# osmocom/osmo-trx

Hardware: AMD Instinct MI355X
Metric: Mbursts/s detect+demod (156.25 sym, 4 SPS) (higher is better)
Workload: dtype f32

## Files before the change

### osmo_trx_amd/csrc/trx_kernel_nb.hip

```cpp
#include "trx_k4_common.h"
#include "trx_nb_asm.inc"

#define NB_D_LEN    160
#define NB_CZ_LEN   (TRX_CZ_PAD + TRX_CORR_NARROW + TRX_CZ_PAD)
#define NB_SLICE    (K4_XS + NB_D_LEN + NB_CZ_LEN)
#define NB_COMP_ROWS (TRX_DELAY_FILTS + 1)
#define NB_TABLES_FLOATS (TRX_SINCV_LDS + 16 * WAVE + NB_COMP_ROWS * 36 + 16 + 8 * 8 + 5 * WAVE + 5 * WAVE + 2 * 8 * 16)
#define NB_TABLES_BYTES (NB_TABLES_FLOATS * 4)
#define NB_WPB 16
#define NB_POOL_RING 64
#define NB_POOL_UNSET (-1)
#define NB_POOL_END (-2)
#define NB_NO_BURST 0xffffffffu
#define NB_LDS_TAIL (16 + 4 * NB_POOL_RING)
#define NB_LDS_BYTES (NB_TABLES_BYTES + NB_WPB * NB_SLICE * 8 + NB_LDS_TAIL)
#define NB_MAX_TOA 32



typedef float v3f __attribute__((ext_vector_type(3)));
typedef int v4i __attribute__((ext_vector_type(4)));
typedef __attribute__((address_space(3))) v2f lds_v2f;

template <typename T>
// ... 160 lines not shown

	uint32_t pre_i[NLD];
	uint32_t pre_prm = 0u;
	auto prefetch = [&](unsigned bb) {
		pre_prm = reinterpret_cast<const uint32_t *>(params)[2 * (size_t)bb];
		const char *src = reinterpret_cast<const char *>(iq + (size_t)bb * 625);
		const uint32_t *const row = reinterpret_cast<const uint32_t *>(src + a_l4);
#pragma unroll
		for (int r = 0; r < NLD - 1; r++)
			pre_i[r] = __builtin_nontemporal_load(row + r * WAVE);
		pre_i[NLD - 1] = __builtin_nontemporal_load(reinterpret_cast<const uint32_t *>(src + a_l4c) + (NLD - 1) * WAVE);
	};
	const unsigned b_first = burst_of((unsigned)wave);
	if (b_first != NB_NO_BURST)
		prefetch(b_first);

	v3f o = { 0.0f, 0.0f, 0.0f };
	int recw = 0;
	int pend_m = 0;
	int pend_rm = 0;
	unsigned pend_b = 0;
	int left_any = 0;
	auto store_pending = [&]() {
		float *const so = soft + (size_t)pend_b * 148;
		int *const rp = reinterpret_cast<int *>(results + pend_b);
		const float oe = o.x;
		asm volatile("s_bfm_b64 exec, 48, 2\n\t"
			     "s_and_b32 exec_lo, exec_lo, %7\n\t"
			     "s_and_b32 exec_hi, exec_hi, %7\n\t"
			     "global_store_dwordx3 %0, %1, %2\n\t"
			     "s_mov_b32 exec_lo, 0\n\t"
			     "s_and_b32 exec_hi, %7, 0x92400000\n\t"
			     "global_store_dword %0, %3, %2\n\t"
			     "s_mov_b32 exec_lo, %8\n\t"
			     "s_mov_b32 exec_hi, 0\n\t"
			     "global_store_dword %4, %5, %6\n\t"
			     "s_mov_b64 exec, -1\n\t"
			     "s_nop 0"
			     :: "v"(a_st), "v"(o), "s"(so), "v"(oe), "v"(a_l4), "v"(recw), "s"(rp), "s"(pend_m), "s"(pend_rm)
			     : "memory", "scc");
	};
	int q_xr = 0, q_xi = 0, q_es = 0, q_toa = 0, q_s = 0, q_fl = 0, q_b = 0;
	int q_n = 0;
	auto flush_records = [&]() {
		const int lane = nb_lane_id();
		if (lane < q_n) {
			const float *const h = lhdr + 8 * (q_fl & 0xff);
			const float xr = __int_as_float(q_xr), xi = __int_as_float(q_xi);
			const float a0 = xr * h[2], a1 = xr * h[3], a2 = xi * h[3], a3 = xi * h[2];
			const float amp_re = a0 - a2, amp_im = a1 + a3;
			const float toa = (float)q_toa * 0.001953125f;
			const float energy = __int_as_float(q_es) * 0.0125f;
			const float rssi = rssi_db(full_scale, energy);
			const float p2 = xi * xi + xr * xr;
			const float C = p2 * h[7];
			const float S = __int_as_float(q_s);
			const float ci = 3.0103f * __log2f(C * __builtin_amdgcn_rcpf(S - C));
			const v4i r0 = { 1, __float_as_int(toa), __float_as_int(amp_re), __float_as_int(amp_im) };
			const v4i r1 = { __float_as_int(ci), __float_as_int(energy), __float_as_int(rssi), q_fl };
			asm volatile("global_store_dwordx4 %0, %1, off\n\t"
				     "global_store_dwordx4 %0, %2, off offset:16\n\t"
				     "s_nop 1"
				     :: "v"(results + (unsigned)q_b), "v"(r0), "v"(r1) : "memory");
		}
		asm volatile("");
		q_n = 0;
	};

	auto queue_record = [&](const int xr_bits, const int xi_bits, const int es_bits, const int toa, const int s_bits, const int fl, const unsigned bb) {
		asm("s_lshl_b64 exec, 1, %[n]\n\t"
		    "v_mov_b32_e32 %[qxr], %[xr]\n\t"
		    "v_mov_b32_e32 %[qxi], %[xi]\n\t"
		    "v_mov_b32_e32 %[qes], %[es]\n\t"
		    "v_mov_b32_e32 %[qtoa], %[toa]\n\t"
		    "v_mov_b32_e32 %[qs], %[ss]\n\t"
		    "v_mov_b32_e32 %[qfl], %[fl]\n\t"
		    "v_mov_b32_e32 %[qb], %[b]\n\t"
		    "s_mov_b64 exec, -1"
		    : [qxr] "+v"(q_xr), [qxi] "+v"(q_xi), [qes] "+v"(q_es), [qtoa] "+v"(q_toa), [qs] "+v"(q_s), [qfl] "+v"(q_fl),
		      [qb] "+v"(q_b)
		    : [n] "s"(uni(q_n)), [xr] "s"(xr_bits), [xi] "s"(xi_bits), [es] "s"(es_bits), [toa] "s"(toa),
		      [ss] "s"(s_bits), [fl] "s"(fl), [b] "s"((int)bb)
		    : "scc");
		q_n++;
	};

	auto demod_general = [&](const int nk, const c32 ampv, const int lane) -> bool {
		constexpr int L = 625, nwrite = 148;
		c32 *const dec = D;
		const trx_tables *tabc = reinterpret_cast<const trx_tables *>(e8_addr - offsetof(trx_tables, edge8));
		asm volatile("" : "+s"(tabc));
		const int w = nk >> 7, fr = nk & 127;
		const int fidx = (fr >= 2) ? (fr >> 1) : TRX_DELAY_FILTS;
		const float ian = __builtin_amdgcn_rcpf(norm2(ampv));
		const c32 scale = make_float2(ampv.x * ian, -ampv.y * ian);
		const int n_lo = w > 0 ? w : 0;
		const int n_hi = (L - 1 + w < 623) ? L - 1 + w : 623;
		const int i_full_lo = cdiv4(n_lo + 15), i_full_hi = fdiv4(n_hi);
		const int i0l = cdiv4(n_lo), i0h = i_full_hi + 1;
		const bool need_lo = (n_hi >= n_lo) && (i0l < i_full_lo) && (i0l < nwrite);
		const bool need_hi = (n_hi >= n_lo) && (i0h <= fdiv4(n_hi + 15)) && (i0h < nwrite);
		if (uni((need_lo && !(n_hi >= 4 * (i_full_lo - 1))) || (need_hi && !((w <= -2) && (n_lo <= 4 * i0h - 15)))))
			return false;
		const int lo_tab = uni(need_lo);
		float ct0 = 0.0f, ct1 = 0.0f, ct2 = 0.0f;
		const int le = lane >> 4, lt = lane & 15;
		const int li = i0l + le;
		const int lt0 = n_lo + 15 - 4 * li;
		const bool lact = lt0 >= 1;
		if (lo_tab) {
			const float *row = &tabc->edge_lo[fidx][(lact ? lt0 : 1) - 1][lt];
			ct0 = row[0];
			ct1 = row[16];
			ct2 = (lt < 4) ? row[32] : 0.0f;
		}
		const int hi_tab = uni(need_hi);
		float ch0 = 0.0f, ch1 = 0.0f, ch2 = 0.0f;
		const int hi_i = i0h + le;
		const int htm = n_hi + 15 - 4 * hi_i;
		const bool hact = htm >= 0;
		if (hi_tab) {
			const float *row = &tabc->edge_hi[fidx][hact ? htm : 0][lt];
			ch0 = row[0];
			ch1 = row[16];
			ch2 = (lt < 4) ? row[32] : 0.0f;
		}
		int tabv = lo_tab | (hi_tab << 1);
		asm volatile("" : "+v"(tabv));
		{
			const int c_full = -24 - w;
			const int i_min = cdiv4(-36 - c_full), i_max = fdiv4(L + 1 - c_full);
			int ic = 3 * lane;
			if (ic < i_min) ic = i_min;
			if (ic > i_max - 2) ic = i_max - 2;
			v2f acc[3];
			asm volatile(NB_ASM_FIRG
				     : [a0] "=&v"(acc[0]), [a1] "=&v"(acc[1]), [a2] "=&v"(acc[2])
				     : [nk] "s"(nk), [pb] "s"(lds_addr(P)), [cb] "s"(lds_addr(comp) + 4u * (K4_U0 + TRX_FUSED_SH)), [kic] "v"(8 * ic)
				     : NB_ASM_CLOBBERS);
			if (n_lo == 0 && lo_tab && i_full_hi >= nwrite - 1) {
				if (lane < 52) {
#pragma unroll
					for (int j = 0; j < 3; j++)
						dec[3 * lane + j] = cmul(make_float2(acc[j].x, acc[j].y), scale);
				}
			} else {
#pragma unroll
				for (int j = 0; j < 3; j++) {
					const int i = 3 * lane + j;
					const bool full = (i >= i_full_lo) && (i <= i_full_hi);
					const c32 d = full ? cmul(make_float2(acc[j].x, acc[j].y), scale) : make_float2(0.0f, 0.0f);
					if (i < 156)
						dec[i] = d;
				}
			}
		}
		const int tab2 = uni(tabv), lo_tab2 = tab2 & 1, hi_tab2 = tab2 & 2;
		if (lo_tab2) {
			const int s0 = 4 * li - 24 - w + lt;
			const c32 *pp = P + ((s0 & 3) * PH_A + PH_M0 + (s0 >> 2));
			const c32 x0 = lds_c32(pp), x1 = lds_c32(pp + 4), x2 = lds_c32(pp + 8);
			float ar = x0.x * ct0, ai = x0.y * ct0;
			ar = fmaf(x1.x, ct1, ar); ai = fmaf(x1.y, ct1, ai);
			ar = fmaf(x2.x, ct2, ar); ai = fmaf(x2.y, ct2, ai);
			const float sr = row_sum(ar), si = row_sum(ai);
			int lt0s = lt0;
			asm volatile("" : "+v"(lt0s));
// ... 105 lines not shown
				int clip;
				asm("s_cmp_lg_u64 %1, 0\n\ts_cselect_b32 %0, 1, 0" : "=s"(clip) : "s"(__ballot(amax > TRX_CLIP_THRESH)) : "scc");

				const int len = 16 + (int)max_toa;
				__builtin_assume(len >= 16 && len <= 16 + NB_MAX_TOA);
				float v;
				const int lag0 = (len <= NB_ASM_CORR_MAX_LEN) ? NB_ASM_CORR_LANE0 : 0;
				asm volatile(NB_ASM_DECCORR
					     : [nrm] "=&v"(v)
					     : [aw] "v"(a_w), [zero] "v"(0), [len] "s"(len), [tsc] "s"(tsc)
					     : NB_ASM_CLOBBERS);
				{
					DIAG_MARK(3);
					int m_bits, es_bits, bidx;
					int kr, ka, kb, kic, ktp;
					asm volatile(NB_ASM_AMAX("ds_read_b32 %[kr], %[l4] offset:%c[lc]", "ds_read_b32 %[ka], %[l4] offset:%c[lc]+256",
								 "ds_read_b32 %[kb], %[l4] offset:%c[lc]+512", "ds_read_b32 %[kic], %[l4] offset:%c[lc]+768",
								 "ds_read_b32 %[ktp], %[l4] offset:%c[lc]+1024", "s_nop 0", "s_nop 0", "s_nop 0")
						     "s_sub_u32 %[bidx], %[bidx], %[lag0]\n\t"
						     "s_waitcnt lgkmcnt(0)"
						     : [m] "=&s"(m_bits), [es] "=&s"(es_bits), [bidx] "=&s"(bidx), [kr] "=&v"(kr), [ka] "=&v"(ka), [kb] "=&v"(kb),
						       [kic] "=&v"(kic), [ktp] "=&v"(ktp)
						     : [nrm] "v"(v), [ep] "v"(epart), [l4] "v"(a_l4), [lag0] "s"(lag0),
						       [lc] "n"((TRX_SINCV_LDS + 16 * WAVE + NB_COMP_ROWS * 36 + 16 + 64 + 5 * WAVE) * 4)
						     : NB_ASM_CLOBBERS);
					DIAG_MARK(4);
					int st, e512;
					float km;
					asm volatile(NB_ASM_DETA
						     : [st] "=&" NB_ASM_ST(st), [e] "=&s"(e512), [km] "=&v"(km)
						     : [bidx] "s"(bidx), [len] "s"(len), [czb] "s"(lds_addr(cz)), [kr] "v"(kr), [ka] "v"(ka), [l16] "v"(a_l16),
						       [gkv] "v"(gkv), [c0] "v"(gc0)
						     : NB_ASM_CLOBBERS_ST);
					DIAG_MARK(5);
					int toa512 = 0, xr_bits = 0, xi_bits = 0;
					if (__builtin_expect(st == 1, 1)) {
						asm volatile(NB_ASM_DETB
							     : [st] "=&" NB_ASM_ST(st), [toa] "=&s"(toa512), [xr] "=&s"(xr_bits), [xi] "=&s"(xi_bits)
							     : [e] "s"(e512), [kb] "v"(kb), [czb] "s"(lds_addr(cz)), [km] "v"(km)
							     : NB_ASM_CLOBBERS_ST);
						DIAG_MARK(6);
					}
					if (__builtin_expect(st != 1, 0)) {
						int stc = st;
						asm volatile("" : "+s"(stc));
						if (stc == 3) {
							const int lane = nb_lane_id();
							if (lane == 0)
								atomicAdd(&g_trx_fast_stats[0], 1ull);
							PeakConst pkc;
							pkc.flA = pkcl[0 * WAVE + lane]; pkc.loA = pkcl[1 * WAVE + lane]; pkc.hiA = pkcl[2 * WAVE + lane];
							pkc.offB = pkcl[3 * WAVE + lane]; pkc.ratio_off = pkcl[4 * WAVE + lane];
							c32 xcorr;
							peak_detect_spec(cz, bidx, sincv, pkc, lane, &toa512, &xcorr, wa4);
							toa512 = uni(toa512);
							xr_bits = uni(__float_as_int(xcorr.x));
							xi_bits = uni(__float_as_int(xcorr.y));
							st = 1;
						} else if (stc == 2) {
							if (nb_lane_id() == 0) atomicAdd(&g_trx_fast_stats[2], 1ull);
							mark_left(b);
							keep = 0;
						} else {
							const float energy = __int_as_float(es_bits) * 0.0125f;
							const float rssi = rssi_db(full_scale, energy);
							const uint32_t flags = ((uint32_t)clip << 8) | (1u << 16);
							int word = clip ? -TRXHIP_SIGERR_CLIP : 0;
							word = put_lane<1>(word, 0.0f);
							word = put_lane<2>(word, 0.0f);
							word = put_lane<3>(word, 0.0f);
							word = put_lane<4>(word, 0.0f);
							word = put_lane<5>(word, energy);
							word = put_lane<6>(word, rssi);
							word = write_lane<7>(word, (int)flags);
							recw = word;
							o = (v3f){ 0.0f, 0.0f, 0.0f };
							pend_rm = 0xff;
						}
					}
					if (__builtin_expect(st == 1, 1)) {
						int ok, s_bits;
						float d0, d1, d2;
						const int t5 = (t5pk << (28 - 4 * tsc)) >> 28;
						asm volatile("s_setprio 0");
						asm volatile(NB_ASM_TAIL
							     : [ok] "=&s"(ok), [ssum] "=&s"(s_bits), [d0] "=&v"(d0), [d1] "=&v"(d1), [d2] "=&v"(d2)
							     : [toa] "s"(toa512), [xr] "s"(xr_bits), [xi] "s"(xi_bits), [t5] "s"(t5), [hdrb] "s"(lds_addr(lhdr) + 32u * (unsigned)tsc),
							       [e8lo] "s"((unsigned)e8_addr), [e8hi] "s"((unsigned)(e8_addr >> 32)), [l16] "v"(a_l16),
							       [aw] "v"(a_w), [pb] "s"(lds_addr(P)), [cb] "s"(lds_addr(comp) + 4u * (K4_U0 + TRX_FUSED_SH)), [db] "s"(lds_addr(D)),
							       [kic] "v"(kic), [ktp] "v"(ktp)
							     : NB_ASM_CLOBBERS);
						DIAG_MARK(10);
						asm volatile("s_setprio 2");
						o.x = __builtin_amdgcn_fmed3f(fmaf(0.5f, d0, 0.5f), 0.0f, 1.0f);
						o.y = __builtin_amdgcn_fmed3f(fmaf(0.5f, d1, 0.5f), 0.0f, 1.0f);
						o.z = __builtin_amdgcn_fmed3f(fmaf(0.5f, d2, 0.5f), 0.0f, 1.0f);
						queue_record(xr_bits, xi_bits, es_bits, toa512 - t5 - 10 * 512, s_bits,
							     (int)((uint32_t)tsc | ((uint32_t)clip << 8) | (37u << 24)), b);
						if (__builtin_expect(!ok, 0)) {
							const int lane = nb_lane_id();
							if (lane == 0) atomicAdd(&g_trx_fast_stats[3], 1ull);
							const float *const h = lhdr + 8 * tsc;
							const float xr = __int_as_float(xr_bits), xi = __int_as_float(xi_bits);
							const float a0 = xr * h[2], a1 = xr * h[3], a2 = xi * h[3], a3 = xi * h[2];
							const c32 ampv = make_float2(unif(a0 - a2), unif(a1 + a3));
							if (!demod_general(t5 + 10 * 512 - toa512, ampv, lane)) {
								q_n--;
								mark_left(b);
								keep = 0;
							}
						}
					}
				}
			}
		}
		pend_b = b;
		pend_m = keep;
		if (__builtin_expect(q_n == WAVE, 0))
			flush_records();
		DIAG_MARK(11);
	}
	asm volatile(NB_ASM_COLD ::: NB_ASM_CLOBBERS);
	store_pending();
	flush_records();
	DIAG_FLUSH();
	if (pooled) {
		__syncthreads();
		int tid0;
		asm volatile("v_mbcnt_lo_u32_b32 %0, -1, 0\n\tv_mbcnt_hi_u32_b32 %0, -1, %0" : "=v"(tid0));
		if (tid0 == 0 && atomicAdd(wg_next + 1, 1) == 0) {
			const unsigned d = __hip_atomic_fetch_add(pool_ctr + 1, 1u, __ATOMIC_ACQ_REL, __HIP_MEMORY_SCOPE_AGENT);
			if (d == gridDim.x - 1u) {
				__hip_atomic_store(pool_ctr, 0u, __ATOMIC_RELAXED, __HIP_MEMORY_SCOPE_AGENT);
				__hip_atomic_store(pool_ctr + 1, 0u, __ATOMIC_RELEASE, __HIP_MEMORY_SCOPE_AGENT);
			}
		}
	}
}
```

### osmo_trx_amd/csrc/trx_nb_asm.inc

```
#define NB_ASM_GDEC_OFF 29968
#define NB_ASM_LSEQ_OFF 32848
#define NB_ASM_DEC_MAX_NACT 60
#define NB_ASM_CORR_LANE0 19
#define NB_ASM_CORR_MAX_LEN 45
#define NB_ASM_AW_PD 512
#define NB_ASM_AW_D 5760
#define NB_ASM_AW_CZ 7136
#define NB_ASM_ST "{s98}"
#define NB_ASM_CLOBBERS "v64", "v65", "v66", "v67", "v68", "v69", "v70", "v71", "v72", "v73", "v74", "v75", "v76", "v77", "v78", "v79", "v80", "v81", "v82", "v83", "v84", "v85", "v86", "v87", "v88", "v89", "v90", "v91", "v92", "v93", "v94", "v95", "v96", "v97", "v98", "v99", "v100", "v101", "v102", "v103", "v104", "v105", "v106", "v107", "v108", "v109", "v110", "v111", "v112", "v113", "v114", "v115", "v116", "v117", "v118", "v119", "v120", "v121", "v122", "v123", "v124", "v125", "v126", "v127", "s87", "s88", "s89", "s90", "s91", "s92", "s93", "s94", "s95", "s96", "s97", "s98", "s99", "vcc", "scc", "memory"
#define NB_ASM_CLOBBERS_ST "v64", "v65", "v66", "v67", "v68", "v69", "v70", "v71", "v72", "v73", "v74", "v75", "v76", "v77", "v78", "v79", "v80", "v81", "v82", "v83", "v84", "v85", "v86", "v87", "v88", "v89", "v90", "v91", "v92", "v93", "v94", "v95", "v96", "v97", "v98", "v99", "v100", "v101", "v102", "v103", "v104", "v105", "v106", "v107", "v108", "v109", "v110", "v111", "v112", "v113", "v114", "v115", "v116", "v117", "v118", "v119", "v120", "v121", "v122", "v123", "v124", "v125", "v126", "v127", "s87", "s88", "s89", "s90", "s91", "s92", "s93", "s94", "s95", "s96", "s97", "s99", "vcc", "scc", "memory"
#define NB_ASM_DECCORR \
	"s_add_u32 s92, %[len], 15\n\t" \
	"s_cmp_gt_u32 %[len], 45\n\t" \
	"s_cbranch_scc1 .Lnbc_dc_wide\n\t" \
	"s_sub_u32 s88, 60, s92\n\t" \
	"s_lshr_b64 exec, -1, s88\n\t" \
	"ds_read_b128 v[120:123], %[zero] offset:29968\n\t" \
	"ds_read_b128 v[124:127], %[zero] offset:29984\n\t" \
	"ds_read_b64 v[98:99], %[aw] offset:1952\n\t" \
	"ds_read_b64 v[100:101], %[aw] offset:3392\n\t" \
	"ds_read_b64 v[102:103], %[aw] offset:4832\n\t" \
	"ds_read_b64 v[96:97], %[aw] offset:512\n\t" \
	"s_waitcnt lgkmcnt(3)\n\t" \
	"v_pk_mul_f32 v[64:65], v[98:99], v[120:121] op_sel:[0,0] op_sel_hi:[1,0]\n\t" \
// ... 1320 lines not shown
	"v_pk_fma_f32 v[64:65], v[84:85], v[98:99], v[64:65] op_sel:[0,0,0] op_sel_hi:[1,0,1]\n\t" \
	"v_pk_fma_f32 v[66:67], v[86:87], v[98:99], v[66:67] op_sel:[0,1,0] op_sel_hi:[1,1,1]\n\t" \
	"ds_read_b64 v[108:109], v69 offset:80\n\t" \
	"ds_read_b32 v122, v72 offset:4096\n\t" \
	"ds_read_b64 v[110:111], v69 offset:88\n\t" \
	"ds_read_b32 v123, v72 offset:6144\n\t" \
	"s_waitcnt lgkmcnt(12)\n\t" \
	"v_pk_fma_f32 v[64:65], v[88:89], v[100:101], v[64:65] op_sel:[0,0,0] op_sel_hi:[1,0,1]\n\t" \
	"v_pk_fma_f32 v[66:67], v[90:91], v[100:101], v[66:67] op_sel:[0,1,0] op_sel_hi:[1,1,1]\n\t" \
	"ds_read_b64 v[112:113], v69 offset:96\n\t" \
	"ds_read_b32 v124, v72 offset:8192\n\t" \
	"ds_read_b64 v[114:115], v69 offset:104\n\t" \
	"ds_read_b32 v125, v72 offset:10240\n\t" \
	"s_waitcnt lgkmcnt(12)\n\t" \
	"v_pk_fma_f32 v[64:65], v[92:93], v[102:103], v[64:65] op_sel:[0,0,0] op_sel_hi:[1,0,1]\n\t" \
	"v_pk_fma_f32 v[66:67], v[94:95], v[102:103], v[66:67] op_sel:[0,1,0] op_sel_hi:[1,1,1]\n\t" \
	"ds_read_b64 v[116:117], v69 offset:112\n\t" \
	"ds_read_b32 v126, v72 offset:12288\n\t" \
	"ds_read_b64 v[118:119], v69 offset:120\n\t" \
	"ds_read_b32 v127, v72 offset:14336\n\t" \
	"s_waitcnt lgkmcnt(12)\n\t" \
	"v_pk_fma_f32 v[64:65], v[104:105], v[120:121], v[64:65] op_sel:[0,0,0] op_sel_hi:[1,0,1]\n\t" \
	"v_pk_fma_f32 v[66:67], v[106:107], v[120:121], v[66:67] op_sel:[0,1,0] op_sel_hi:[1,1,1]\n\t" \
	"s_waitcnt lgkmcnt(8)\n\t" \
	"v_pk_fma_f32 v[64:65], v[108:109], v[122:123], v[64:65] op_sel:[0,0,0] op_sel_hi:[1,0,1]\n\t" \
	"v_pk_fma_f32 v[66:67], v[110:111], v[122:123], v[66:67] op_sel:[0,1,0] op_sel_hi:[1,1,1]\n\t" \
	"s_waitcnt lgkmcnt(4)\n\t" \
	"v_pk_fma_f32 v[64:65], v[112:113], v[124:125], v[64:65] op_sel:[0,0,0] op_sel_hi:[1,0,1]\n\t" \
	"v_pk_fma_f32 v[66:67], v[114:115], v[124:125], v[66:67] op_sel:[0,1,0] op_sel_hi:[1,1,1]\n\t" \
	"s_waitcnt lgkmcnt(0)\n\t" \
	"v_pk_fma_f32 v[64:65], v[116:117], v[126:127], v[64:65] op_sel:[0,0,0] op_sel_hi:[1,0,1]\n\t" \
	"v_pk_fma_f32 v[66:67], v[118:119], v[126:127], v[66:67] op_sel:[0,1,0] op_sel_hi:[1,1,1]\n\t" \
	"s_mov_b64 exec, -1\n\t" \
	"v_pk_add_f32 v[74:75], v[64:65], v[66:67]\n\t" \
	"s_add_u32 s92, %[e], 497\n\t" \
	"v_pk_mul_f32 v[76:77], v[74:75], v[74:75]\n\t" \
	"s_mov_b32 s98, 1\n\t" \
	"v_add_f32_e32 v78, v77, v76\n\t" \
	"v_fmamk_f32 v79, v78, 0x36c9539c, %[km]\n\t" \
	"v_sub_f32_e32 v96, v78, v79\n\t" \
	"v_add_f32_e32 v97, v78, v79\n\t" \
	"s_nop 0\n\t" \
	"v_mov_b32_dpp v96, v96 quad_perm:[1,0,3,2] row_mask:0xf bank_mask:0xf\n\t" \
	"v_cmp_lt_f32_e64 s[88:89], v97, v96\n\t" \
	"s_lshr_b32 s90, s88, 1\n\t" \
	"s_or_b32 s90, s90, s88\n\t" \
	"s_and_b32 s91, s90, 0x15555555\n\t" \
	"s_cmp_eq_u32 s91, 0x15555555\n\t" \
	"s_cbranch_scc0 .Lnbc_db_careful\n\t" \
	"s_mov_b32 s94, 0\n\t" \
	"s_lshl1_add_u32 s95, s94, 0\n\t" \
	"s_bitcmp1_b32 s88, s95\n\t" \
	"s_addc_u32 s94, s94, s94\n\t" \
	"s_lshl1_add_u32 s95, s94, 2\n\t" \
	"s_bitcmp1_b32 s88, s95\n\t" \
	"s_addc_u32 s94, s94, s94\n\t" \
	"s_lshl1_add_u32 s95, s94, 6\n\t" \
	"s_bitcmp1_b32 s88, s95\n\t" \
	"s_addc_u32 s94, s94, s94\n\t" \
	"s_lshl1_add_u32 s95, s94, 14\n\t" \
	"s_bitcmp1_b32 s88, s95\n\t" \
	"s_addc_u32 s94, s94, s94\n\t" \
	".Lnb_db_walked:\n\t" \
	"s_add_u32 s93, s94, 32\n\t" \
	"s_lshl1_add_u32 %[toa], s94, s92\n\t" \
	"v_readlane_b32 %[xr], v74, s93\n\t" \
	"v_readlane_b32 %[xi], v75, s93\n\t" \
	".Lnb_db_end:\n\t"
#define NB_ASM_TAIL \
	"v_mov_b32_e32 v65, %[hdrb]\n\t" \
	"ds_read_b128 v[68:71], v65\n\t" \
	"s_sub_u32 s88, %[t5], %[toa]\n\t" \
	"s_add_u32 s87, s88, 5120\n\t" \
	"s_mov_b32 %[ok], 0\n\t" \
	"s_and_b32 s91, s87, 127\n\t" \
	"s_lshr_b32 s92, s91, 1\n\t" \
	"s_cmp_ge_u32 s91, 2\n\t" \
	"s_cselect_b32 s92, s92, 64\n\t" \
	"s_mul_i32 s93, s92, 768\n\t" \
	"s_add_u32 s94, %[e8lo], s93\n\t" \
	"s_addc_u32 s95, %[e8hi], 0\n\t" \
	"s_abs_i32 s96, %[toa]\n\t" \
	"s_add_u32 s96, s96, 256\n\t" \
	"global_load_dwordx4 v[120:123], %[l16], s[94:95]\n\t" \
	"s_lshr_b32 s96, s96, 9\n\t" \
	"s_sub_u32 s97, 0, s96\n\t" \
	"s_cmp_lt_i32 %[toa], 0\n\t" \
	"s_cselect_b32 s96, s97, s96\n\t" \
	"s_lshl_b32 s96, s96, 3\n\t" \
	"v_add_u32_e32 v64, s96, %[aw]\n\t" \
	"s_bfm_b64 exec, 16, 0\n\t" \
	"ds_read_b64 v[66:67], v64 offset:5760\n\t" \
	"s_mov_b64 exec, -1\n\t" \
	"s_waitcnt lgkmcnt(1)\n\t" \
	"v_mul_f32_e32 v82, %[xr], v70\n\t" \
	"v_mul_f32_e32 v83, %[xr], v71\n\t" \
	"v_mul_f32_e32 v84, %[xi], v71\n\t" \
	"v_mul_f32_e32 v85, %[xi], v70\n\t" \
	"v_sub_f32_e32 v86, v82, v84\n\t" \
	"v_add_f32_e32 v87, v83, v85\n\t" \
	"v_mul_f32_e32 v90, v86, v86\n\t" \
	"v_mul_f32_e32 v89, v87, v87\n\t" \
	"v_add_f32_e32 v89, v89, v90\n\t" \
	"v_rcp_f32_e32 v89, v89\n\t" \
	"s_mov_b32 s88, 0xaaaaaaaa\n\t" \
	"s_mov_b32 s89, 0xaaaaaaaa\n\t" \
	"v_mul_f32_e32 v91, v86, v89\n\t" \
	"v_mul_f32_e64 v92, -v87, v89\n\t" \
	"v_cndmask_b32_e64 v119, v91, v92, s[88:89]\n\t" \
	"s_mov_b32 s88, 0xcccccccc\n\t" \
	"s_mov_b32 s89, 0xcccccccc\n\t" \
	"v_cndmask_b32_e64 v119, v119, -v119, s[88:89]\n\t" \
	"s_bfm_b64 exec, 16, 0\n\t" \
	"s_waitcnt lgkmcnt(0)\n\t" \
	"v_pk_mul_f32 v[66:67], v[66:67], v[66:67]\n\t" \
	"s_ashr_i32 s88, s87, 7\n\t" \
	"v_add_f32_e32 v81, v67, v66\n\t" \
	"s_and_b32 s89, s87, 127\n\t" \
	"s_lshr_b32 s90, s89, 1\n\t" \
	"v_add_f32_dpp v81, v81, v81 quad_perm:[1,0,3,2] row_mask:0xf bank_mask:0xf\n\t" \
	"s_cmp_ge_u32 s89, 2\n\t" \
	"s_cselect_b32 s90, s90, 64\n\t" \
	"v_add_f32_dpp v81, v81, v81 quad_perm:[2,3,0,1] row_mask:0xf bank_mask:0xf\n\t" \
	"s_sub_u32 s91, -18, s88\n\t" \
	"s_and_b32 s92, s91, 3\n\t" \
	"v_add_f32_dpp v81, v81, v81 row_half_mirror row_mask:0xf bank_mask:0xf\n\t" \
	"s_ashr_i32 s93, s91, 2\n\t" \
	"s_mul_i32 s94, s92, 180\n\t" \
	"v_add_f32_dpp v81, v81, v81 row_mirror row_mask:0xf bank_mask:0xf\n\t" \
	"s_add_u32 s94, s94, s93\n\t" \
	"s_lshl3_add_u32 s94, s94, %[pb]\n\t" \
	"v_mul_f32_e32 v81, 0x3d800000, v81\n\t" \
	"s_mul_i32 s95, s90, 144\n\t" \
	"s_add_u32 s95, s95, %[cb]\n\t" \
	"v_readlane_b32 %[ssum], v81, 0\n\t" \
	"s_mov_b64 exec, -1\n\t" \
	"s_sub_u32 s96, 0, s88\n\t" \
	"s_cmp_gt_u32 s96, 36\n\t" \
	"s_cbranch_scc1 .Lnbc_tl_wait\n\t" \
	"s_mov_b32 %[ok], 1\n\t" \
	"v_add_u32_e32 v112, s94, %[kic]\n\t" \
	"s_add_u32 s96, s92, 1\n\t" \
	"s_lshr_b32 s96, s96, 2\n\t" \
	"s_mul_i32 s96, s96, -5752\n\t" \
	"s_add_u32 s96, s96, 1440\n\t" \
	"v_add_u32_e32 v113, s96, v112\n\t" \
	"s_add_u32 s96, s92, 2\n\t" \
	"s_lshr_b32 s96, s96, 2\n\t" \
	"s_mul_i32 s96, s96, -5752\n\t" \
	"s_add_u32 s96, s96, 2880\n\t" \
	"v_add_u32_e32 v114, s96, v112\n\t" \
	"s_add_u32 s96, s92, 3\n\t" \
	"s_lshr_b32 s96, s96, 2\n\t" \
	"s_mul_i32 s96, s96, -5752\n\t" \
	"s_add_u32 s96, s96, 4320\n\t" \
	"v_add_u32_e32 v115, s96, v112\n\t" \
	"ds_read_b64 v[72:73], v112 offset:96\n\t" \
	"ds_read_b64 v[74:75], v113 offset:96\n\t" \
	"ds_read_b64 v[76:77], v114 offset:96\n\t" \
	"ds_read_b64 v[78:79], v115 offset:96\n\t" \
	"ds_read_b64 v[80:81], v112 offset:104\n\t" \
	"ds_read_b64 v[82:83], v113 offset:104\n\t" \
	"ds_read_b64 v[84:85], v114 offset:104\n\t" \
	"ds_read_b64 v[86:87], v115 offset:104\n\t" \
	"ds_read_b64 v[88:89], v112 offset:112\n\t" \
	"ds_read_b64 v[90:91], v113 offset:112\n\t" \
	"ds_read_b64 v[92:93], v114 offset:112\n\t" \
	"ds_read_b64 v[94:95], v115 offset:112\n\t" \
	"v_add_u32_e32 v116, %[db], %[l16]\n\t" \
	"v_cmp_lt_i32_e32 vcc, -1, %[ktp]\n\t" \
	"v_add_u32_e32 v117, %[db], %[ktp]\n\t" \
	"v_mov_b32_e32 v118, s95\n\t" \
	"v_mov_b64_e32 v[64:65], 0\n\t" \
	"v_mov_b64_e32 v[66:67], 0\n\t" \
	"v_mov_b64_e32 v[68:69], 0\n\t" \
	"v_cndmask_b32_e32 v117, v118, v117, vcc\n\t" \
	"s_waitcnt vmcnt(0)\n\t" \
	"ds_write_b128 v116, v[120:123]\n\t" \
	"ds_read_b128 v[96:99], v117 offset:0\n\t" \
	"ds_read_b128 v[100:103], v117 offset:16\n\t" \
	"ds_read_b128 v[104:107], v117 offset:32\n\t" \
	"ds_read_b128 v[108:111], v117 offset:48\n\t" \
	"ds_read_b128 v[124:127], v117 offset:64\n\t" \
	"s_waitcnt lgkmcnt(4)\n\t" \
	"ds_read_b128 v[120:123], v117 offset:80\n\t" \
	"v_pk_fma_f32 v[64:65], v[72:73], v[96:97], v[64:65] op_sel:[0,0,0] op_sel_hi:[1,0,1]\n\t" \
	"v_pk_fma_f32 v[66:67], v[80:81], v[96:97], v[66:67] op_sel:[0,0,0] op_sel_hi:[1,0,1]\n\t" \
	"v_pk_fma_f32 v[68:69], v[88:89], v[96:97], v[68:69] op_sel:[0,0,0] op_sel_hi:[1,0,1]\n\t" \
	"v_pk_fma_f32 v[64:65], v[74:75], v[96:97], v[64:65] op_sel:[0,1,0] op_sel_hi:[1,1,1]\n\t" \
	"v_pk_fma_f32 v[66:67], v[82:83], v[96:97], v[66:67] op_sel:[0,1,0] op_sel_hi:[1,1,1]\n\t" \
	"v_pk_fma_f32 v[68:69], v[90:91], v[96:97], v[68:69] op_sel:[0,1,0] op_sel_hi:[1,1,1]\n\t" \
	"v_pk_fma_f32 v[64:65], v[76:77], v[98:99], v[64:65] op_sel:[0,0,0] op_sel_hi:[1,0,1]\n\t" \
	"v_pk_fma_f32 v[66:67], v[84:85], v[98:99], v[66:67] op_sel:[0,0,0] op_sel_hi:[1,0,1]\n\t" \
	"v_pk_fma_f32 v[68:69], v[92:93], v[98:99], v[68:69] op_sel:[0,0,0] op_sel_hi:[1,0,1]\n\t" \
	"v_pk_fma_f32 v[64:65], v[78:79], v[98:99], v[64:65] op_sel:[0,1,0] op_sel_hi:[1,1,1]\n\t" \
	"v_pk_fma_f32 v[66:67], v[86:87], v[98:99], v[66:67] op_sel:[0,1,0] op_sel_hi:[1,1,1]\n\t" \
	"v_pk_fma_f32 v[68:69], v[94:95], v[98:99], v[68:69] op_sel:[0,1,0] op_sel_hi:[1,1,1]\n\t" \
	"s_waitcnt lgkmcnt(4)\n\t" \
	"v_pk_fma_f32 v[64:65], v[80:81], v[100:101], v[64:65] op_sel:[0,0,0] op_sel_hi:[1,0,1]\n\t" \
	"v_pk_fma_f32 v[66:67], v[88:89], v[100:101], v[66:67] op_sel:[0,0,0] op_sel_hi:[1,0,1]\n\t" \
	"v_mov_b32_dpp v68, v68 wave_shr:1 row_mask:0xf bank_mask:0xf bound_ctrl:0\n\t" \
	"v_mov_b32_dpp v69, v69 wave_shr:1 row_mask:0xf bank_mask:0xf bound_ctrl:0\n\t" \
	"v_pk_fma_f32 v[64:65], v[82:83], v[100:101], v[64:65] op_sel:[0,1,0] op_sel_hi:[1,1,1]\n\t" \
	"v_pk_fma_f32 v[66:67], v[90:91], v[100:101], v[66:67] op_sel:[0,1,0] op_sel_hi:[1,1,1]\n\t" \
	"v_pk_fma_f32 v[68:69], v[72:73], v[100:101], v[68:69] op_sel:[0,0,0] op_sel_hi:[1,0,1]\n\t" \
	"v_pk_fma_f32 v[64:65], v[84:85], v[102:103], v[64:65] op_sel:[0,0,0] op_sel_hi:[1,0,1]\n\t" \
	"v_pk_fma_f32 v[66:67], v[92:93], v[102:103], v[66:67] op_sel:[0,0,0] op_sel_hi:[1,0,1]\n\t" \
	"v_pk_fma_f32 v[68:69], v[74:75], v[100:101], v[68:69] op_sel:[0,1,0] op_sel_hi:[1,1,1]\n\t" \
	"v_pk_fma_f32 v[64:65], v[86:87], v[102:103], v[64:65] op_sel:[0,1,0] op_sel_hi:[1,1,1]\n\t" \
	"v_pk_fma_f32 v[66:67], v[94:95], v[102:103], v[66:67] op_sel:[0,1,0] op_sel_hi:[1,1,1]\n\t" \
	"v_pk_fma_f32 v[68:69], v[76:77], v[102:103], v[68:69] op_sel:[0,0,0] op_sel_hi:[1,0,1]\n\t" \
	"s_waitcnt lgkmcnt(3)\n\t" \
	"v_pk_fma_f32 v[64:65], v[88:89], v[104:105], v[64:65] op_sel:[0,0,0] op_sel_hi:[1,0,1]\n\t" \
	"s_bfm_b64 exec, 52, 0\n\t" \
	"v_mov_b32_dpp v66, v66 wave_shr:1 row_mask:0xf bank_mask:0xf bound_ctrl:0\n\t" \
	"v_mov_b32_dpp v67, v67 wave_shr:1 row_mask:0xf bank_mask:0xf bound_ctrl:0\n\t" \
	"s_mov_b64 exec, -1\n\t" \
	"v_pk_fma_f32 v[68:69], v[78:79], v[102:103], v[68:69] op_sel:[0,1,0] op_sel_hi:[1,1,1]\n\t" \
	"v_pk_fma_f32 v[64:65], v[90:91], v[104:105], v[64:65] op_sel:[0,1,0] op_sel_hi:[1,1,1]\n\t" \
	"v_pk_fma_f32 v[66:67], v[72:73], v[104:105], v[66:67] op_sel:[0,0,0] op_sel_hi:[1,0,1]\n\t" \
	"v_pk_fma_f32 v[68:69], v[80:81], v[104:105], v[68:69] op_sel:[0,0,0] op_sel_hi:[1,0,1]\n\t" \
	"v_pk_fma_f32 v[64:65], v[92:93], v[106:107], v[64:65] op_sel:[0,0,0] op_sel_hi:[1,0,1]\n\t" \
	"v_pk_fma_f32 v[66:67], v[74:75], v[104:105], v[66:67] op_sel:[0,1,0] op_sel_hi:[1,1,1]\n\t" \
	"v_pk_fma_f32 v[68:69], v[82:83], v[104:105], v[68:69] op_sel:[0,1,0] op_sel_hi:[1,1,1]\n\t" \
	"v_pk_fma_f32 v[64:65], v[94:95], v[106:107], v[64:65] op_sel:[0,1,0] op_sel_hi:[1,1,1]\n\t" \
	"v_pk_fma_f32 v[66:67], v[76:77], v[106:107], v[66:67] op_sel:[0,0,0] op_sel_hi:[1,0,1]\n\t" \
	"v_pk_fma_f32 v[68:69], v[84:85], v[106:107], v[68:69] op_sel:[0,0,0] op_sel_hi:[1,0,1]\n\t" \
	"v_mov_b32_dpp v64, v64 wave_shr:1 row_mask:0xf bank_mask:0xf bound_ctrl:0\n\t" \
	"v_mov_b32_dpp v65, v65 wave_shr:1 row_mask:0xf bank_mask:0xf bound_ctrl:0\n\t" \
	"v_pk_fma_f32 v[66:67], v[78:79], v[106:107], v[66:67] op_sel:[0,1,0] op_sel_hi:[1,1,1]\n\t" \
	"v_pk_fma_f32 v[68:69], v[86:87], v[106:107], v[68:69] op_sel:[0,1,0] op_sel_hi:[1,1,1]\n\t" \
	"s_waitcnt lgkmcnt(2)\n\t" \
	"v_pk_fma_f32 v[64:65], v[72:73], v[108:109], v[64:65] op_sel:[0,0,0] op_sel_hi:[1,0,1]\n\t" \
	"v_pk_fma_f32 v[66:67], v[80:81], v[108:109], v[66:67] op_sel:[0,0,0] op_sel_hi:[1,0,1]\n\t" \
	"v_pk_fma_f32 v[68:69], v[88:89], v[108:109], v[68:69] op_sel:[0,0,0] op_sel_hi:[1,0,1]\n\t" \
	"v_pk_fma_f32 v[64:65], v[74:75], v[108:109], v[64:65] op_sel:[0,1,0] op_sel_hi:[1,1,1]\n\t" \
	"v_pk_fma_f32 v[66:67], v[82:83], v[108:109], v[66:67] op_sel:[0,1,0] op_sel_hi:[1,1,1]\n\t" \
	"v_pk_fma_f32 v[68:69], v[90:91], v[108:109], v[68:69] op_sel:[0,1,0] op_sel_hi:[1,1,1]\n\t" \
	"v_pk_fma_f32 v[64:65], v[76:77], v[110:111], v[64:65] op_sel:[0,0,0] op_sel_hi:[1,0,1]\n\t" \
	"v_pk_fma_f32 v[66:67], v[84:85], v[110:111], v[66:67] op_sel:[0,0,0] op_sel_hi:[1,0,1]\n\t" \
	"v_pk_fma_f32 v[68:69], v[92:93], v[110:111], v[68:69] op_sel:[0,0,0] op_sel_hi:[1,0,1]\n\t" \
	"v_pk_fma_f32 v[64:65], v[78:79], v[110:111], v[64:65] op_sel:[0,1,0] op_sel_hi:[1,1,1]\n\t" \
	"v_pk_fma_f32 v[66:67], v[86:87], v[110:111], v[66:67] op_sel:[0,1,0] op_sel_hi:[1,1,1]\n\t" \
	"v_pk_fma_f32 v[68:69], v[94:95], v[110:111], v[68:69] op_sel:[0,1,0] op_sel_hi:[1,1,1]\n\t" \
	"s_waitcnt lgkmcnt(1)\n\t" \
	"v_pk_fma_f32 v[64:65], v[80:81], v[124:125], v[64:65] op_sel:[0,0,0] op_sel_hi:[1,0,1]\n\t" \
	"v_pk_fma_f32 v[66:67], v[88:89], v[124:125], v[66:67] op_sel:[0,0,0] op_sel_hi:[1,0,1]\n\t" \
	"v_mov_b32_dpp v68, v68 wave_shr:1 row_mask:0xf bank_mask:0xf bound_ctrl:0\n\t" \
	"v_mov_b32_dpp v69, v69 wave_shr:1 row_mask:0xf bank_mask:0xf bound_ctrl:0\n\t" \
	"v_pk_fma_f32 v[64:65], v[82:83], v[124:125], v[64:65] op_sel:[0,1,0] op_sel_hi:[1,1,1]\n\t" \
	"v_pk_fma_f32 v[66:67], v[90:91], v[124:125], v[66:67] op_sel:[0,1,0] op_sel_hi:[1,1,1]\n\t" \
	"v_pk_fma_f32 v[68:69], v[72:73], v[124:125], v[68:69] op_sel:[0,0,0] op_sel_hi:[1,0,1]\n\t" \
	"v_pk_fma_f32 v[64:65], v[84:85], v[126:127], v[64:65] op_sel:[0,0,0] op_sel_hi:[1,0,1]\n\t" \
	"v_pk_fma_f32 v[66:67], v[92:93], v[126:127], v[66:67] op_sel:[0,0,0] op_sel_hi:[1,0,1]\n\t" \
	"v_pk_fma_f32 v[68:69], v[74:75], v[124:125], v[68:69] op_sel:[0,1,0] op_sel_hi:[1,1,1]\n\t" \
	"v_pk_fma_f32 v[64:65], v[86:87], v[126:127], v[64:65] op_sel:[0,1,0] op_sel_hi:[1,1,1]\n\t" \
	"v_pk_fma_f32 v[66:67], v[94:95], v[126:127], v[66:67] op_sel:[0,1,0] op_sel_hi:[1,1,1]\n\t" \
	"v_pk_fma_f32 v[68:69], v[76:77], v[126:127], v[68:69] op_sel:[0,0,0] op_sel_hi:[1,0,1]\n\t" \
	"s_waitcnt lgkmcnt(0)\n\t" \
	"v_pk_fma_f32 v[64:65], v[88:89], v[120:121], v[64:65] op_sel:[0,0,0] op_sel_hi:[1,0,1]\n\t" \
	"s_bfm_b64 exec, 52, 0\n\t" \
	"v_mov_b32_dpp v66, v66 wave_shr:1 row_mask:0xf bank_mask:0xf bound_ctrl:0\n\t" \
	"v_mov_b32_dpp v67, v67 wave_shr:1 row_mask:0xf bank_mask:0xf bound_ctrl:0\n\t" \
	"s_mov_b64 exec, -1\n\t" \
	"v_pk_fma_f32 v[68:69], v[78:79], v[126:127], v[68:69] op_sel:[0,1,0] op_sel_hi:[1,1,1]\n\t" \
	"v_pk_fma_f32 v[64:65], v[90:91], v[120:121], v[64:65] op_sel:[0,1,0] op_sel_hi:[1,1,1]\n\t" \
	"v_pk_fma_f32 v[66:67], v[72:73], v[120:121], v[66:67] op_sel:[0,0,0] op_sel_hi:[1,0,1]\n\t" \
	"v_pk_fma_f32 v[68:69], v[80:81], v[120:121], v[68:69] op_sel:[0,0,0] op_sel_hi:[1,0,1]\n\t" \
	"v_pk_fma_f32 v[64:65], v[92:93], v[122:123], v[64:65] op_sel:[0,0,0] op_sel_hi:[1,0,1]\n\t" \
	"v_pk_fma_f32 v[66:67], v[74:75], v[120:121], v[66:67] op_sel:[0,1,0] op_sel_hi:[1,1,1]\n\t" \
	"v_pk_fma_f32 v[68:69], v[82:83], v[120:121], v[68:69] op_sel:[0,1,0] op_sel_hi:[1,1,1]\n\t" \
	"v_pk_fma_f32 v[64:65], v[94:95], v[122:123], v[64:65] op_sel:[0,1,0] op_sel_hi:[1,1,1]\n\t" \
	"v_pk_fma_f32 v[66:67], v[76:77], v[122:123], v[66:67] op_sel:[0,0,0] op_sel_hi:[1,0,1]\n\t" \
	"v_pk_fma_f32 v[68:69], v[84:85], v[122:123], v[68:69] op_sel:[0,0,0] op_sel_hi:[1,0,1]\n\t" \
	"v_mov_b32_dpp v64, v64 wave_shr:1 row_mask:0xf bank_mask:0xf bound_ctrl:0\n\t" \
	"v_mov_b32_dpp v65, v65 wave_shr:1 row_mask:0xf bank_mask:0xf bound_ctrl:0\n\t" \
	"v_pk_fma_f32 v[66:67], v[78:79], v[122:123], v[66:67] op_sel:[0,1,0] op_sel_hi:[1,1,1]\n\t" \
	"v_pk_fma_f32 v[68:69], v[86:87], v[122:123], v[68:69] op_sel:[0,1,0] op_sel_hi:[1,1,1]\n\t" \
	"s_mov_b32 exec_lo, 0\n\t" \
	"s_mov_b32 exec_hi, 0xfff00000\n\t" \
	"v_pk_add_f32 v[64:65], v[64:65], v[66:67]\n\t" \
	"s_mov_b64 exec, -1\n\t" \
	"v_mul_f32_dpp %[d1], v119, v66 quad_perm:[3,2,1,0] row_mask:0xf bank_mask:0xf\n\t" \
	"v_mul_f32_dpp %[d2], v119, v68 quad_perm:[0,3,2,1] row_mask:0xf bank_mask:0xf\n\t" \
	"v_mul_f32_dpp %[d0], v119, v64 quad_perm:[2,1,0,3] row_mask:0xf bank_mask:0xf\n\t" \
	"v_fmac_f32_dpp %[d1], v119, v67 quad_perm:[2,1,0,3] row_mask:0xf bank_mask:0xf\n\t" \
	"v_fmac_f32_dpp %[d2], v119, v69 quad_perm:[3,2,1,0] row_mask:0xf bank_mask:0xf\n\t" \
	"v_fmac_f32_dpp %[d0], v119, v65 quad_perm:[1,0,3,2] row_mask:0xf bank_mask:0xf\n\t" \
	".Lnb_tl_end:\n\t"
#define NB_ASM_FIRG \
	"s_ashr_i32 s88, %[nk], 7\n\t" \
	"s_and_b32 s89, %[nk], 127\n\t" \
	"s_lshr_b32 s90, s89, 1\n\t" \
	"s_cmp_ge_u32 s89, 2\n\t" \
	"s_cselect_b32 s90, s90, 64\n\t" \
	"s_sub_u32 s91, -18, s88\n\t" \
	"s_and_b32 s92, s91, 3\n\t" \
	"s_ashr_i32 s93, s91, 2\n\t" \
	"s_mul_i32 s94, s92, 180\n\t" \
	"s_add_u32 s94, s94, s93\n\t" \
	"s_lshl3_add_u32 s94, s94, %[pb]\n\t" \
	"s_mul_i32 s95, s90, 144\n\t" \
	"s_add_u32 s95, s95, %[cb]\n\t" \
	"v_add_u32_e32 v112, s94, %[kic]\n\t" \
	"s_add_u32 s96, s92, 1\n\t" \
	"s_lshr_b32 s96, s96, 2\n\t" \
	"s_mul_i32 s96, s96, -5752\n\t" \
	"s_add_u32 s96, s96, 1440\n\t" \
	"v_add_u32_e32 v113, s96, v112\n\t" \
	"s_add_u32 s96, s92, 2\n\t" \
	"s_lshr_b32 s96, s96, 2\n\t" \
	"s_mul_i32 s96, s96, -5752\n\t" \
	"s_add_u32 s96, s96, 2880\n\t" \
	"v_add_u32_e32 v114, s96, v112\n\t" \
	"s_add_u32 s96, s92, 3\n\t" \
	"s_lshr_b32 s96, s96, 2\n\t" \
	"s_mul_i32 s96, s96, -5752\n\t" \
	"s_add_u32 s96, s96, 4320\n\t" \
	"v_add_u32_e32 v115, s96, v112\n\t" \
	"v_mov_b64_e32 %[a0], 0\n\t" \
	"v_mov_b64_e32 %[a1], 0\n\t" \
	"v_mov_b64_e32 %[a2], 0\n\t" \
	"v_mov_b32_e32 v117, s95\n\t" \
	"s_bfm_b64 exec, 52, 0\n\t" \
	"ds_read_b64 v[72:73], v112 offset:96\n\t" \
	"ds_read_b64 v[74:75], v113 offset:96\n\t" \
	"ds_read_b64 v[76:77], v114 offset:96\n\t" \
	"ds_read_b64 v[78:79], v115 offset:96\n\t" \
	"ds_read_b64 v[80:81], v112 offset:104\n\t" \
	"ds_read_b64 v[82:83], v113 offset:104\n\t" \
	"ds_read_b64 v[84:85], v114 offset:104\n\t" \
	"ds_read_b64 v[86:87], v115 offset:104\n\t" \
	"ds_read_b64 v[88:89], v112 offset:112\n\t" \
	"ds_read_b64 v[90:91], v113 offset:112\n\t" \
	"ds_read_b64 v[92:93], v114 offset:112\n\t" \
	"ds_read_b64 v[94:95], v115 offset:112\n\t" \
	"ds_read_b128 v[104:107], v117\n\t" \
	"ds_read_b128 v[108:111], v117 offset:16\n\t" \
	"ds_read_b64 v[96:97], v112 offset:120\n\t" \
	"ds_read_b64 v[98:99], v113 offset:120\n\t" \
	"ds_read_b64 v[100:101], v114 offset:120\n\t" \
	"ds_read_b64 v[102:103], v115 offset:120\n\t" \
// ... 196 lines not shown
```

Measured before the change: 1147.

## Load tail taps directly into registers per lane and fuse record queueing into asm

The tail asm used to load a 16-byte global chunk, write it to LDS, wait, and then read six 128-bit values back from LDS. Now lanes 52-63 load the six values straight from global memory into registers, lanes 0-51 read them from LDS, and the write-then-read round trip through LDS is gone. The per-burst record queue moves are also placed inside the asm block between the loads and the single wait, so they hide load latency, and the scalar queue_record call now runs only on the rare fallback path. The risk is that the merged wait removes the staggered lgkmcnt overlap, and the exec-mask split relies on how ktp and the LDS base are laid out per lane.

```diff
diff --git a/osmo_trx_amd/csrc/trx_kernel_nb.hip b/osmo_trx_amd/csrc/trx_kernel_nb.hip
--- a/osmo_trx_amd/csrc/trx_kernel_nb.hip
+++ b/osmo_trx_amd/csrc/trx_kernel_nb.hip
@@ -266,7 +266,6 @@
 		    : [n] "s"(uni(q_n)), [xr] "s"(xr_bits), [xi] "s"(xi_bits), [es] "s"(es_bits), [toa] "s"(toa),
 		      [ss] "s"(s_bits), [fl] "s"(fl), [b] "s"((int)bb)
 		    : "scc");
-		q_n++;
 	};
 
 	auto demod_general = [&](const int nk, const c32 ampv, const int lane) -> bool {
@@ -538,22 +537,24 @@
 						int ok, s_bits;
 						float d0, d1, d2;
 						const int t5 = (t5pk << (28 - 4 * tsc)) >> 28;
+						const int rec_fl = (int)((uint32_t)tsc | ((uint32_t)clip << 8) | (37u << 24));
 						asm volatile("s_setprio 0");
 						asm volatile(NB_ASM_TAIL
-							     : [ok] "=&s"(ok), [ssum] "=&s"(s_bits), [d0] "=&v"(d0), [d1] "=&v"(d1), [d2] "=&v"(d2)
+							     : [ok] "=&s"(ok), [ssum] "=&s"(s_bits), [d0] "=&v"(d0), [d1] "=&v"(d1), [d2] "=&v"(d2),
+							       [qxr] "+v"(q_xr), [qxi] "+v"(q_xi), [qes] "+v"(q_es), [qtoa] "+v"(q_toa), [qs] "+v"(q_s), [qfl] "+v"(q_fl),
+							       [qb] "+v"(q_b)
 							     : [toa] "s"(toa512), [xr] "s"(xr_bits), [xi] "s"(xi_bits), [t5] "s"(t5), [hdrb] "s"(lds_addr(lhdr) + 32u * (unsigned)tsc),
-							       [e8lo] "s"((unsigned)e8_addr), [e8hi] "s"((unsigned)(e8_addr >> 32)), [l16] "v"(a_l16),
-							       [aw] "v"(a_w), [pb] "s"(lds_addr(P)), [cb] "s"(lds_addr(comp) + 4u * (K4_U0 + TRX_FUSED_SH)), [db] "s"(lds_addr(D)),
-							       [kic] "v"(kic), [ktp] "v"(ktp)
+							       [e8lo] "s"((unsigned)e8_addr), [e8hi] "s"((unsigned)(e8_addr >> 32)),
+							       [aw] "v"(a_w), [pb] "s"(lds_addr(P)), [cb] "s"(lds_addr(comp) + 4u * (K4_U0 + TRX_FUSED_SH)),
+							       [kic] "v"(kic), [ktp] "v"(ktp), [es] "s"(es_bits), [fl] "s"(rec_fl), [bi] "s"((int)b), [qn] "s"(uni(q_n))
 							     : NB_ASM_CLOBBERS);
 						DIAG_MARK(10);
 						asm volatile("s_setprio 2");
 						o.x = __builtin_amdgcn_fmed3f(fmaf(0.5f, d0, 0.5f), 0.0f, 1.0f);
 						o.y = __builtin_amdgcn_fmed3f(fmaf(0.5f, d1, 0.5f), 0.0f, 1.0f);
 						o.z = __builtin_amdgcn_fmed3f(fmaf(0.5f, d2, 0.5f), 0.0f, 1.0f);
-						queue_record(xr_bits, xi_bits, es_bits, toa512 - t5 - 10 * 512, s_bits,
-							     (int)((uint32_t)tsc | ((uint32_t)clip << 8) | (37u << 24)), b);
 						if (__builtin_expect(!ok, 0)) {
+							queue_record(xr_bits, xi_bits, es_bits, toa512 - t5 - 10 * 512, s_bits, rec_fl, b);
 							const int lane = nb_lane_id();
 							if (lane == 0) atomicAdd(&g_trx_fast_stats[3], 1ull);
 							const float *const h = lhdr + 8 * tsc;
@@ -566,6 +567,7 @@
 								keep = 0;
 							}
 						}
+						q_n++;
 					}
 				}
 			}
diff --git a/osmo_trx_amd/csrc/trx_nb_asm.inc b/osmo_trx_amd/csrc/trx_nb_asm.inc
--- a/osmo_trx_amd/csrc/trx_nb_asm.inc
+++ b/osmo_trx_amd/csrc/trx_nb_asm.inc
@@ -1426,7 +1426,15 @@
 	"s_addc_u32 s95, %[e8hi], 0\n\t" \
 	"s_abs_i32 s96, %[toa]\n\t" \
 	"s_add_u32 s96, s96, 256\n\t" \
-	"global_load_dwordx4 v[120:123], %[l16], s[94:95]\n\t" \
+	"s_mov_b32 exec_lo, 0\n\t" \
+	"s_mov_b32 exec_hi, 0xfff00000\n\t" \
+	"global_load_dwordx4 v[96:99], %[ktp], s[94:95]\n\t" \
+	"global_load_dwordx4 v[100:103], %[ktp], s[94:95] offset:16\n\t" \
+	"global_load_dwordx4 v[104:107], %[ktp], s[94:95] offset:32\n\t" \
+	"global_load_dwordx4 v[108:111], %[ktp], s[94:95] offset:48\n\t" \
+	"global_load_dwordx4 v[124:127], %[ktp], s[94:95] offset:64\n\t" \
+	"global_load_dwordx4 v[120:123], %[ktp], s[94:95] offset:80\n\t" \
+	"s_mov_b64 exec, -1\n\t" \
 	"s_lshr_b32 s96, s96, 9\n\t" \
 	"s_sub_u32 s97, 0, s96\n\t" \
 	"s_cmp_lt_i32 %[toa], 0\n\t" \
@@ -1499,6 +1507,7 @@
 	"s_mul_i32 s96, s96, -5752\n\t" \
 	"s_add_u32 s96, s96, 4320\n\t" \
 	"v_add_u32_e32 v115, s96, v112\n\t" \
+	"v_mov_b32_e32 v118, s95\n\t" \
 	"ds_read_b64 v[72:73], v112 offset:96\n\t" \
 	"ds_read_b64 v[74:75], v113 offset:96\n\t" \
 	"ds_read_b64 v[76:77], v114 offset:96\n\t" \
@@ -1511,23 +1520,28 @@
 	"ds_read_b64 v[90:91], v113 offset:112\n\t" \
 	"ds_read_b64 v[92:93], v114 offset:112\n\t" \
 	"ds_read_b64 v[94:95], v115 offset:112\n\t" \
-	"v_add_u32_e32 v116, %[db], %[l16]\n\t" \
-	"v_cmp_lt_i32_e32 vcc, -1, %[ktp]\n\t" \
-	"v_add_u32_e32 v117, %[db], %[ktp]\n\t" \
-	"v_mov_b32_e32 v118, s95\n\t" \
+	"s_bfm_b64 exec, 52, 0\n\t" \
+	"ds_read_b128 v[96:99], v118\n\t" \
+	"ds_read_b128 v[100:103], v118 offset:16\n\t" \
+	"ds_read_b128 v[104:107], v118 offset:32\n\t" \
+	"ds_read_b128 v[108:111], v118 offset:48\n\t" \
+	"ds_read_b128 v[124:127], v118 offset:64\n\t" \
+	"ds_read_b128 v[120:123], v118 offset:80\n\t" \
+	"s_mov_b64 exec, -1\n\t" \
 	"v_mov_b64_e32 v[64:65], 0\n\t" \
 	"v_mov_b64_e32 v[66:67], 0\n\t" \
 	"v_mov_b64_e32 v[68:69], 0\n\t" \
-	"v_cndmask_b32_e32 v117, v118, v117, vcc\n\t" \
-	"s_waitcnt vmcnt(0)\n\t" \
-	"ds_write_b128 v116, v[120:123]\n\t" \
-	"ds_read_b128 v[96:99], v117 offset:0\n\t" \
-	"ds_read_b128 v[100:103], v117 offset:16\n\t" \
-	"ds_read_b128 v[104:107], v117 offset:32\n\t" \
-	"ds_read_b128 v[108:111], v117 offset:48\n\t" \
-	"ds_read_b128 v[124:127], v117 offset:64\n\t" \
-	"s_waitcnt lgkmcnt(4)\n\t" \
-	"ds_read_b128 v[120:123], v117 offset:80\n\t" \
+	"s_sub_u32 s97, 0, s87\n\t" \
+	"s_lshl_b64 exec, 1, %[qn]\n\t" \
+	"v_mov_b32_e32 %[qxr], %[xr]\n\t" \
+	"v_mov_b32_e32 %[qxi], %[xi]\n\t" \
+	"v_mov_b32_e32 %[qes], %[es]\n\t" \
+	"v_mov_b32_e32 %[qtoa], s97\n\t" \
+	"v_mov_b32_e32 %[qs], %[ssum]\n\t" \
+	"v_mov_b32_e32 %[qfl], %[fl]\n\t" \
+	"v_mov_b32_e32 %[qb], %[bi]\n\t" \
+	"s_mov_b64 exec, -1\n\t" \
+	"s_waitcnt vmcnt(0) lgkmcnt(0)\n\t" \
 	"v_pk_fma_f32 v[64:65], v[72:73], v[96:97], v[64:65] op_sel:[0,0,0] op_sel_hi:[1,0,1]\n\t" \
 	"v_pk_fma_f32 v[66:67], v[80:81], v[96:97], v[66:67] op_sel:[0,0,0] op_sel_hi:[1,0,1]\n\t" \
 	"v_pk_fma_f32 v[68:69], v[88:89], v[96:97], v[68:69] op_sel:[0,0,0] op_sel_hi:[1,0,1]\n\t" \
@@ -1540,7 +1554,6 @@
 	"v_pk_fma_f32 v[64:65], v[78:79], v[98:99], v[64:65] op_sel:[0,1,0] op_sel_hi:[1,1,1]\n\t" \
 	"v_pk_fma_f32 v[66:67], v[86:87], v[98:99], v[66:67] op_sel:[0,1,0] op_sel_hi:[1,1,1]\n\t" \
 	"v_pk_fma_f32 v[68:69], v[94:95], v[98:99], v[68:69] op_sel:[0,1,0] op_sel_hi:[1,1,1]\n\t" \
-	"s_waitcnt lgkmcnt(4)\n\t" \
 	"v_pk_fma_f32 v[64:65], v[80:81], v[100:101], v[64:65] op_sel:[0,0,0] op_sel_hi:[1,0,1]\n\t" \
 	"v_pk_fma_f32 v[66:67], v[88:89], v[100:101], v[66:67] op_sel:[0,0,0] op_sel_hi:[1,0,1]\n\t" \
 	"v_mov_b32_dpp v68, v68 wave_shr:1 row_mask:0xf bank_mask:0xf bound_ctrl:0\n\t" \
@@ -1554,7 +1567,6 @@
 	"v_pk_fma_f32 v[64:65], v[86:87], v[102:103], v[64:65] op_sel:[0,1,0] op_sel_hi:[1,1,1]\n\t" \
 	"v_pk_fma_f32 v[66:67], v[94:95], v[102:103], v[66:67] op_sel:[0,1,0] op_sel_hi:[1,1,1]\n\t" \
 	"v_pk_fma_f32 v[68:69], v[76:77], v[102:103], v[68:69] op_sel:[0,0,0] op_sel_hi:[1,0,1]\n\t" \
-	"s_waitcnt lgkmcnt(3)\n\t" \
 	"v_pk_fma_f32 v[64:65], v[88:89], v[104:105], v[64:65] op_sel:[0,0,0] op_sel_hi:[1,0,1]\n\t" \
 	"s_bfm_b64 exec, 52, 0\n\t" \
 	"v_mov_b32_dpp v66, v66 wave_shr:1 row_mask:0xf bank_mask:0xf bound_ctrl:0\n\t" \
@@ -1574,7 +1586,6 @@
 	"v_mov_b32_dpp v65, v65 wave_shr:1 row_mask:0xf bank_mask:0xf bound_ctrl:0\n\t" \
 	"v_pk_fma_f32 v[66:67], v[78:79], v[106:107], v[66:67] op_sel:[0,1,0] op_sel_hi:[1,1,1]\n\t" \
 	"v_pk_fma_f32 v[68:69], v[86:87], v[106:107], v[68:69] op_sel:[0,1,0] op_sel_hi:[1,1,1]\n\t" \
-	"s_waitcnt lgkmcnt(2)\n\t" \
 	"v_pk_fma_f32 v[64:65], v[72:73], v[108:109], v[64:65] op_sel:[0,0,0] op_sel_hi:[1,0,1]\n\t" \
 	"v_pk_fma_f32 v[66:67], v[80:81], v[108:109], v[66:67] op_sel:[0,0,0] op_sel_hi:[1,0,1]\n\t" \
 	"v_pk_fma_f32 v[68:69], v[88:89], v[108:109], v[68:69] op_sel:[0,0,0] op_sel_hi:[1,0,1]\n\t" \
@@ -1587,7 +1598,6 @@
 	"v_pk_fma_f32 v[64:65], v[78:79], v[110:111], v[64:65] op_sel:[0,1,0] op_sel_hi:[1,1,1]\n\t" \
 	"v_pk_fma_f32 v[66:67], v[86:87], v[110:111], v[66:67] op_sel:[0,1,0] op_sel_hi:[1,1,1]\n\t" \
 	"v_pk_fma_f32 v[68:69], v[94:95], v[110:111], v[68:69] op_sel:[0,1,0] op_sel_hi:[1,1,1]\n\t" \
-	"s_waitcnt lgkmcnt(1)\n\t" \
 	"v_pk_fma_f32 v[64:65], v[80:81], v[124:125], v[64:65] op_sel:[0,0,0] op_sel_hi:[1,0,1]\n\t" \
 	"v_pk_fma_f32 v[66:67], v[88:89], v[124:125], v[66:67] op_sel:[0,0,0] op_sel_hi:[1,0,1]\n\t" \
 	"v_mov_b32_dpp v68, v68 wave_shr:1 row_mask:0xf bank_mask:0xf bound_ctrl:0\n\t" \
@@ -1601,7 +1611,6 @@
 	"v_pk_fma_f32 v[64:65], v[86:87], v[126:127], v[64:65] op_sel:[0,1,0] op_sel_hi:[1,1,1]\n\t" \
 	"v_pk_fma_f32 v[66:67], v[94:95], v[126:127], v[66:67] op_sel:[0,1,0] op_sel_hi:[1,1,1]\n\t" \
 	"v_pk_fma_f32 v[68:69], v[76:77], v[126:127], v[68:69] op_sel:[0,0,0] op_sel_hi:[1,0,1]\n\t" \
-	"s_waitcnt lgkmcnt(0)\n\t" \
 	"v_pk_fma_f32 v[64:65], v[88:89], v[120:121], v[64:65] op_sel:[0,0,0] op_sel_hi:[1,0,1]\n\t" \
 	"s_bfm_b64 exec, 52, 0\n\t" \
 	"v_mov_b32_dpp v66, v66 wave_shr:1 row_mask:0xf bank_mask:0xf bound_ctrl:0\n\t" \
```

Result: no change. 1153, median of 6 (+0.5%).
